# tjiangHIT/cuteSV

Measured on NVIDIA H100. Metric: sv_signatures_clustered_per_sec, higher is better.
Workload: dtype int32

## Files before the change

cutesv_b200/csrc/cutesv_b200.cu:

```cuda
#include <cuda_runtime.h>
#include <dlfcn.h>
#include <nccl.h>
#include <stdarg.h>
#include <stdio.h>
#include <stdlib.h>
#include <string.h>

#include <algorithm>
#include <atomic>
#include <string>
#include <vector>

#include "../../include/cutesv_b200.h"
#include "core.h"
#include "devprims.cuh"
#include "host_tables.h"
#include "kernels.cuh"
#include "radix.cuh"
#include "extract.cuh"
#include "scan_core.h"
#include "sa_core.h"

using namespace csv;

// ... 932 lines not shown
    return CSV_OK;
}
template <typename K>
static int lane_sort(csv_ctx* c, Lane& L, bool iota, int64_t n, int bits, K** keys_out, uint32_t** vals_out) {
    return radix_sort<K>(c, L.stream, L.hist, c->lb, L.lb_status, true, L.keys_a.as<K>(), L.vals_a.as<uint32_t>(), L.keys_b.as<K>(),
                         L.vals_b.as<uint32_t>(), iota, n, bits, keys_out, vals_out);
}

static ClusterParams cluster_params(const csv_params& P, int t) {
    ClusterParams C;
    C.min_support = P.min_support;
    C.min_support_allele = P.min_support_allele;
    C.min_size = P.min_size;
    C.max_size = P.max_size;
    C.bias = t == CSV_DEL ? P.bias_del : t == CSV_INS ? P.bias_ins : t == CSV_INV ? P.bias_inv : t == CSV_DUP ? P.bias_dup : P.bias_tra;
    C.ratio = t == CSV_DEL ? P.ratio_del : t == CSV_INS ? P.ratio_ins : P.ratio_tra;
    C.keep = P.remain_reads_ratio > 1 ? 1 : P.remain_reads_ratio;
    C.genotype = P.genotype;
    return C;
}

static Emit make_emit(csv_ctx* c) {
    Emit E;
    E.cand = c->cand_tmp.as<csv_cand>();
    E.names = c->names.as<int32_t>();
    E.cnt = c->cnt.as<uint32_t>();
    E.ctr = c->counters.as<Counters>();
    E.pow_half = c->pow_half.as<double>();
    E.lim.cap_cand = c->cap_cand;
    E.lim.cap_names = c->cap_names;
    E.lim.pow_n = c->pow_n;
    E.cursor = c->emit_cursor.as<unsigned long long>();
    return E;
}

static int run_segment_and_cluster(csv_ctx* c, Lane& L, TypeJob& J, int t, uint32_t kslot_base) {
    Counters* ctr = c->counters.as<Counters>();
    const cudaStream_t s = L.stream;
    stage_begin(c, s, CSV_ST_SEGMENT);
    J.kslot_base = kslot_base;
    J.kept_start = c->kept[t].as<uint32_t>();
    J.big_list = L.big_list.as<uint32_t>();
    J.giant_list = L.giant_list.as<uint32_t>();
    J.giant_arena = L.giant_arena.as<char>();
    J.big_cap = (uint32_t)(L.big_list.cap / 4);
    J.giant_cap = (uint32_t)(L.giant_list.cap / 4);
    TileSync ts;
    int rc = make_sync(c->lb, L.lb_status, s, (size_t)(J.n_host / SEL_TILE + 2), &ts);
    if (rc) return rc;
    if ((J.cp.min_support + 31) / 32 + 1 <= HEAD_MAX_NEED_WORDS) {
        MemberRec MR;
        memset(&MR, 0, sizeof(MR));
        J.small_list = nullptr; J.n_small = nullptr; J.rest_list = nullptr; J.n_rest = nullptr; J.n_rest_lo = nullptr;
        if ((t == CSV_DEL || t == CSV_INS) && J.iv.rec) {
            MR.rec = const_cast<IndelRec*>(J.iv.rec); MR.recc = const_cast<int32_t*>(J.iv.recc);
            MR.a = J.iv.a; MR.b = J.iv.b; MR.rid = J.iv.rid; MR.c = J.iv.recc ? J.iv.c : nullptr; MR.sidx = J.iv.sidx;
            if (t == CSV_DEL && J.keys32) { MR.del_off = c->d_off.as<uint64_t>(); MR.n_contigs = c->n_contigs; }
            if (J.cp.keep >= 1.0 && J.small_path) {
                CU(L.rest_list.ensure((size_t)c->kept_cap[t] * 12 + 64));
                MR.rest_list = L.rest_list.as<uint32_t>();
                MR.small_list = (uint2*)(L.rest_list.as<uint32_t>() + c->kept_cap[t] + (c->kept_cap[t] & 1u));
                if ((rc = take_ticket(c->lb, &MR.n_small)) || (rc = take_ticket(c->lb, &MR.n_rest)) || (rc = take_ticket(c->lb, &MR.n_rest_lo)))
                    return rc;
                MR.rest_cap = c->kept_cap[t];
                J.small_list = MR.small_list; J.n_small = MR.n_small; J.rest_list = MR.rest_list; J.n_rest = MR.n_rest;
                J.n_rest_lo = MR.n_rest_lo; J.rest_cap = MR.rest_cap;
            }
        }
        const int sel_grid = std::min(grid_for(c, J.n_host, SEL_TILE, 64), resident_grid(c, k_select_heads, SEL_THREADS, 0));
        if (L.prev_is_chain_kernel)
            LAUNCH_PDL(c, s, k_select_heads, sel_grid, SEL_THREADS, 0, J, c->kept[t].as<uint32_t>(), c->kept_cap[t],
                       &ctr->n_kept[t], ts, &ctr->status, (uint32_t)ST_LIST_OVERFLOW, MR);
        else
            LAUNCH(c, s, k_select_heads, sel_grid, SEL_THREADS, 0, J, c->kept[t].as<uint32_t>(), c->kept_cap[t],
                   &ctr->n_kept[t], ts, &ctr->status, (uint32_t)ST_LIST_OVERFLOW, MR);
    } else {
        J.iv.rec = nullptr; J.iv.recc = nullptr;
        HeadPred hp{J};
        LAUNCH(c, s, (k_select<HeadPred>), grid_for(c, J.n_host, SEL_TILE, 4), SEL_THREADS, 0, hp, J.n_host, J.n_dev,
               c->kept[t].as<uint32_t>(), c->kept_cap[t], &ctr->n_kept[t], ts, &ctr->status, (uint32_t)ST_LIST_OVERFLOW);
    }
    stage_end(c, s, CSV_ST_SEGMENT);
    stage_begin(c, s, CSV_ST_CLUSTER);
    Emit E = make_emit(c);
    const size_t smem_warp = (size_t)(CL_THREADS / 32) * WARP_M * ARENA_PER_MAX + (CL_THREADS / 32) * 40 * 8;
    uint32_t* work = nullptr;
    if ((rc = take_ticket(c->lb, &work))) return rc;
    const bool keep_all = J.cp.keep >= 1.0;
    const int side_k = t == CSV_INS ? 1 : 0;
    cudaStream_t gs = s;
    if (kind_of(t) == 0 && keep_all && J.small_path) {
        uint32_t* work_s = nullptr;
        if ((rc = take_ticket(c->lb, &work_s))) return rc;
        TypeJob JS = J;
        uint32_t* n_rest = nullptr;
        if (!J.small_list) {
            CU(L.rest_list.ensure((size_t)c->kept_cap[t] * 12 + 64));
            if ((rc = take_ticket(c->lb, &n_rest))) return rc;
            JS.rest_list = L.rest_list.as<uint32_t>();
            JS.n_rest = n_rest;
        } else if (!c->profiling) {
            gs = c->side_stream[side_k];
            CU(cudaEventRecord(c->ev_side_fork[side_k], s));
            CU(cudaStreamWaitEvent(gs, c->ev_side_fork[side_k], 0));
        }
        if (t == CSV_INS) LAUNCH_PDL_NAMED(c, s, "k_cluster_small<INS>", (k_cluster_small<true>), c->n_sm * 6, 256, 0, JS, E, ctr, work_s, n_rest);
        else LAUNCH_PDL_NAMED(c, s, "k_cluster_small<DEL>", (k_cluster_small<false>), c->n_sm * 6, 256, 0, JS, E, ctr, work_s, n_rest);
        if (!J.small_list) { J.rest_list = JS.rest_list; J.n_rest = n_rest; }
    } else { J.small_list = nullptr; J.n_small = nullptr; J.rest_list = nullptr; J.n_rest = nullptr; J.n_rest_lo = nullptr; }
    switch (kind_of(t)) {
        case 0:
            if (t == CSV_DEL) { if (keep_all) launch_cluster_kind<6, 0>(c, gs, J, E, ctr, work, smem_warp); else launch_cluster_kind<4, 0>(c, gs, J, E, ctr, work, smem_warp); }
            else { if (keep_all) launch_cluster_kind<7, 0>(c, gs, J, E, ctr, work, smem_warp); else launch_cluster_kind<5, 0>(c, gs, J, E, ctr, work, smem_warp); }
            break;
        case 1: launch_cluster_kind<1, 1>(c, gs, J, E, ctr, work, smem_warp); break;
        case 2: launch_cluster_kind<2, 2>(c, gs, J, E, ctr, work, smem_warp); break;
        default: launch_cluster_kind<3, 3>(c, gs, J, E, ctr, work, smem_warp); break;
    }
    if (gs != s) {
        CU(cudaEventRecord(c->ev_side_join[side_k], gs));
        CU(cudaStreamWaitEvent(s, c->ev_side_join[side_k], 0));
    }
    stage_end(c, s, CSV_ST_CLUSTER);
    if (L.mark >= 0) { CU(cudaEventRecord(c->kivs[L.mark].b, s)); L.mark = -1; }
    return CSV_OK;
}

static int run_indel(csv_ctx* c, Lane& L, int t, uint32_t kslot_base) {
    SigTable& s = c->sig[t];
    const cudaStream_t st = L.stream;
    const int64_t n = s.n;
    const uint64_t total = c->contig_off[c->n_contigs];
    const int bits = bits_for(total);
    const bool k64 = bits > 32;
    ContigTab ct{c->d_off.as<uint64_t>(), c->d_len_eff.as<int64_t>(), c->n_contigs};
    Counters* ctr = c->counters.as<Counters>();
    TypeJob J;
    memset(&J, 0, sizeof(J));
    J.svtype = t; J.n_host = n; J.n_dev = nullptr;
    J.cp = cluster_params(c->P, t);
    const uint32_t radius = (uint32_t)std::min<int64_t>((int64_t)(J.cp.min_support - 1) * J.cp.bias, 1 << 24);
    const double lambda = (double)n * (2.0 * radius + 2.0 * (1 << BKT_SHIFT)) / (double)std::max<uint64_t>(total, 1);
    const int rb = (int)((radius + (1u << BKT_SHIFT) - 1) >> BKT_SHIFT);
    const bool prefilter = !k64 && c->prefilter_enabled && J.cp.min_support >= 3 && lambda < 0.8 * J.cp.min_support &&
                           n >= (1 << 16) && rb <= BKT_PAD;
    J.iv.rec = nullptr; J.iv.recc = nullptr;
    uint32_t* sidx = nullptr;
    int rc;
    if (prefilter) {
        int W = PART_W_MAX;
        while (W > PART_W_MIN && (int64_t)(total >> W) + 1 < 2 * (int64_t)c->n_sm) W--;
        const int P = (int)(total >> W) + 1;
        const int n_chunks = (int)((n + PART_ROUND - 1) / PART_ROUND);
        const size_t run_words = (size_t)(P + 1) * n_chunks, edge_words = (size_t)P * 2 * BKT_PAD;
        stage_begin(c, st, CSV_ST_KEYS);
        CU(L.boff.ensure((run_words + edge_words) * 4));
        uint32_t* runs = L.boff.as<uint32_t>();
        uint32_t* edge = runs + run_words;
        CU(L.rec_a.ensure((size_t)n * sizeof(IndelRec)));
        CU(cudaMemsetAsync(edge, 0, edge_words * 4, st));
        const int is_ins = t == CSV_INS ? 1 : 0;
        if ((((uintptr_t)s.chrom.p) | ((uintptr_t)s.a.p)) & 15)
            return set_err(CSV_E_STATE, "signature columns are not 16 B aligned");
        uint2* pairs = (uint2*)L.keys_a.p;
        LAUNCH(c, st, k_part_scatter, n_chunks, PS_THREADS, ps_smem_bytes(), s.chrom.as<int32_t>(), s.a.as<int32_t>(), n, is_ins, ct, W, P,
               n_chunks, rb, pairs, runs, edge, &ctr->status);
        stage_end(c, st, CSV_ST_KEYS);
        stage_begin(c, st, CSV_ST_SORT);
        TileSync ts;
        rc = make_sync(c->lb, L.lb_status, st, (size_t)P, &ts);
        if (rc) return rc;
        uint32_t* n_pass = &ctr->n_dom[t];
        const size_t smem = pf_smem_bytes(W);
        const int g = std::min(P, resident_grid(c, k_part_filter, 256, smem));
        LAUNCH_PDL(c, st, k_part_filter, g, 256, smem, (const uint2*)pairs, (const uint32_t*)runs, n_chunks, P, W, rb, (uint32_t)J.cp.min_support,
                   (const uint32_t*)edge, L.keys_b.as<uint32_t>(), L.vals_b.as<uint32_t>(), (uint2*)L.rec_a.p, n_pass, ts);
        stage_end(c, st, CSV_ST_SORT);
        if (c->lane_marks) {
            kprof_begin(c, st, t == CSV_DEL ? "back end<DEL>" : "back end<INS>");
            L.mark = (int)c->kivs.size() - 1;
        }
        J.n_dev = n_pass;
        J.keys32 = L.keys_b.as<uint32_t>();
        sidx = L.vals_b.as<uint32_t>();
    } else {
        stage_begin(c, st, CSV_ST_KEYS);
        if (!k64)
            LAUNCH(c, st, (k_indel_keys<uint32_t>), grid_for(c, n, 256), 256, 0, s.chrom.as<int32_t>(), s.a.as<int32_t>(), s.b.as<int32_t>(),
                   s.rid.as<int32_t>(), n, t == CSV_INS ? 1 : 0, ct, L.keys_a.as<uint32_t>(), &ctr->status);
        else
            LAUNCH(c, st, (k_indel_keys<uint64_t>), grid_for(c, n, 256), 256, 0, s.chrom.as<int32_t>(), s.a.as<int32_t>(), s.b.as<int32_t>(),
                   s.rid.as<int32_t>(), n, t == CSV_INS ? 1 : 0, ct, L.keys_a.as<uint64_t>(), &ctr->status);
        stage_end(c, st, CSV_ST_KEYS);
        stage_begin(c, st, CSV_ST_SORT);
        if (!k64) {
            uint32_t* ko = nullptr;
            rc = lane_sort<uint32_t>(c, L, true, n, bits, &ko, &sidx);
            J.keys32 = ko;
        } else {
            uint64_t* ko = nullptr;
            rc = lane_sort<uint64_t>(c, L, true, n, bits, &ko, &sidx);
            J.keys64 = ko;
        }
        if (rc) return rc;
        stage_end(c, st, CSV_ST_SORT);
    }
    J.iv.chrom = s.chrom.as<int32_t>(); J.iv.a = s.a.as<int32_t>(); J.iv.b = s.b.as<int32_t>(); J.iv.rid = s.rid.as<int32_t>();
    J.iv.c = s.has_c ? s.c.as<int32_t>() : nullptr;
    J.iv.sidx = sidx;
    if (!k64 && c->records_enabled && (J.cp.min_support + 31) / 32 + 1 <= HEAD_MAX_NEED_WORDS) {
        const bool with_c = t == CSV_INS && s.has_c;
        CU(L.rec_a.ensure((size_t)n * sizeof(IndelRec)));
        if (with_c) CU(L.recc_a.ensure((size_t)n * 4));
        J.iv.rec = L.rec_a.as<IndelRec>();
        J.iv.recc = with_c ? L.recc_a.as<int32_t>() : nullptr;
    }
    J.iv.is_ins = t == CSV_INS ? 1 : 0;
    J.small_path = c->small_path_enabled ? 1 : 0;
    L.prev_is_chain_kernel = prefilter;
    rc = run_segment_and_cluster(c, L, J, t, kslot_base);
    L.prev_is_chain_kernel = false;
    return rc;
}

static int run_other(csv_ctx* c, Lane& L, int t, uint32_t kslot_base) {
    SigTable& s = c->sig[t];
    const cudaStream_t st = L.stream;
    const int64_t n = s.n;
    SmallWork& w = L.small;
    ContigTab ct{c->d_off.as<uint64_t>(), c->d_len_eff.as<int64_t>(), c->n_contigs};
    Counters* ctr = c->counters.as<Counters>();
    const uint64_t hi_max = t == CSV_DUP ? (uint64_t)c->n_contigs : t == CSV_INV ? 2ull * c->n_contigs : 4ull * c->n_contigs * c->n_contigs;
    const int clog = c->n_contigs > 1 ? bits_for((uint64_t)c->n_contigs - 1) : 0;
    const bool compact = t == CSV_TRA && 2 * clog + 33 > 64;
    const int prim_bits = 31 + bits_for(compact ? (uint64_t)n : hi_max);
    const int32_t* col_c = s.has_c ? s.c.as<int32_t>() : nullptr;
    const bool chain = c->small_chain[t];
    uint64_t* k_prim = chain ? w.k_prim.as<uint64_t>() : L.keys_a.as<uint64_t>();
    int rc;
    stage_begin(c, st, CSV_ST_KEYS);
    if (!compact) {
        LAUNCH(c, st, (k_other_keys<false>), grid_for(c, n, 256), 256, 0, s.chrom.as<int32_t>(), s.a.as<int32_t>(), s.b.as<int32_t>(),
               s.rid.as<int32_t>(), col_c, n, t, ct, chain ? w.k_rid.as<uint32_t>() : (uint32_t*)nullptr, w.k_b.as<uint32_t>(), k_prim,
               &ctr->status);
    } else {
        LAUNCH(c, st, (k_other_keys<true>), grid_for(c, n, 256), 256, 0, s.chrom.as<int32_t>(), s.a.as<int32_t>(), s.b.as<int32_t>(),
               s.rid.as<int32_t>(), col_c, n, t, ct, chain ? w.k_rid.as<uint32_t>() : (uint32_t*)nullptr, w.k_b.as<uint32_t>(),
               L.keys_a.as<uint64_t>(), &ctr->status);
        uint64_t* pair_sorted = nullptr;
        uint32_t* pair_perm = nullptr;
        rc = lane_sort<uint64_t>(c, L, true, n, bits_for(hi_max), &pair_sorted, &pair_perm);
        if (rc) return rc;
        uint32_t* rank = w.sel.as<uint32_t>();
        LAUNCH(c, st, k_tra_pair_flags, grid_for(c, n, 256), 256, 0, (const uint64_t*)pair_sorted, n, rank);
        TileSync ts;
        rc = make_sync(c->lb, L.lb_status, st, (size_t)(n / (SEL_THREADS * 4) + 2), &ts);
        if (rc) return rc;
        LAUNCH(c, st, (k_scan_excl<4>), grid_for(c, n, SEL_THREADS * 4, 4), SEL_THREADS, 0, rank, n, (const uint32_t*)nullptr,
               (const uint32_t*)nullptr, (uint32_t*)nullptr, ts);
        LAUNCH(c, st, k_tra_compact_key, grid_for(c, n, 256), 256, 0, (const uint32_t*)pair_perm, (const uint32_t*)rank, s.a.as<int32_t>(), n,
               k_prim);
    }
    stage_end(c, st, CSV_ST_KEYS);
    stage_begin(c, st, CSV_ST_SORT);
    if (!chain) {
        uint64_t* k64o = nullptr;
        uint32_t* perm = nullptr;
        rc = lane_sort<uint64_t>(c, L, true, n, prim_bits, &k64o, &perm);
        if (rc) return rc;
        LAUNCH(c, st, k_run_fixup, grid_for(c, n, 256), 256, 0, k64o, perm, n, s.b.as<int32_t>(), s.rid.as<int32_t>(), w.perm_b.as<uint32_t>(),
               &ctr->status);
    } else {
        uint32_t *k32o = nullptr, *perm = nullptr;
        LAUNCH(c, st, (k_gather_keys<uint32_t>), grid_for(c, n, 256), 256, 0, w.k_rid.as<uint32_t>(), (const uint32_t*)nullptr, n, L.keys_a.as<uint32_t>());
        rc = lane_sort<uint32_t>(c, L, true, n, 31, &k32o, &perm);
        if (rc) return rc;
        CU(cudaMemcpyAsync(w.perm_a.p, perm, (size_t)n * 4, cudaMemcpyDeviceToDevice, st));
        LAUNCH(c, st, (k_gather_keys<uint32_t>), grid_for(c, n, 256), 256, 0, w.k_b.as<uint32_t>(), w.perm_a.as<uint32_t>(), n, L.keys_a.as<uint32_t>());
        CU(cudaMemcpyAsync(L.vals_a.p, w.perm_a.p, (size_t)n * 4, cudaMemcpyDeviceToDevice, st));
        rc = lane_sort<uint32_t>(c, L, false, n, 31, &k32o, &perm);
        if (rc) return rc;
        CU(cudaMemcpyAsync(w.perm_a.p, perm, (size_t)n * 4, cudaMemcpyDeviceToDevice, st));
        LAUNCH(c, st, (k_gather_keys<uint64_t>), grid_for(c, n, 256), 256, 0, w.k_prim.as<uint64_t>(), w.perm_a.as<uint32_t>(), n, L.keys_a.as<uint64_t>());
        CU(cudaMemcpyAsync(L.vals_a.p, w.perm_a.p, (size_t)n * 4, cudaMemcpyDeviceToDevice, st));
        uint64_t* k64o = nullptr;
        rc = lane_sort<uint64_t>(c, L, false, n, prim_bits, &k64o, &perm);
        if (rc) return rc;
        CU(cudaMemcpyAsync(w.perm_b.p, perm, (size_t)n * 4, cudaMemcpyDeviceToDevice, st));
    }
    stage_end(c, st, CSV_ST_SORT);
    stage_begin(c, st, CSV_ST_SEGMENT);
    uint32_t* n_u = &ctr->n_dom[t];
    TileSync ts;
    rc = make_sync(c->lb, L.lb_status, st, (size_t)(n / SEL_TILE + 2), &ts);
    if (rc) return rc;
    DedupPred dp{s.chrom.as<int32_t>(), s.a.as<int32_t>(), s.b.as<int32_t>(), s.rid.as<int32_t>(), col_c, w.perm_b.as<uint32_t>()};
    LAUNCH(c, st, (k_select<DedupPred>), grid_for(c, n, SEL_TILE, 4), SEL_THREADS, 0, dp, n, (const uint32_t*)nullptr, w.sel.as<uint32_t>(),
           (uint32_t)n, n_u, ts, &ctr->status, (uint32_t)ST_INTERNAL);
    LAUNCH(c, st, k_other_gather, grid_for(c, n, 256), 256, 0, s.chrom.as<int32_t>(), s.a.as<int32_t>(), s.b.as<int32_t>(), s.rid.as<int32_t>(),
           col_c, w.perm_b.as<uint32_t>(), w.sel.as<uint32_t>(), n_u, w.u_chrom.as<int32_t>(), w.u_a.as<int32_t>(), w.u_b.as<int32_t>(),
           w.u_rid.as<int32_t>(), w.u_c.as<int32_t>());
    stage_end(c, st, CSV_ST_SEGMENT);
    TypeJob J;
    memset(&J, 0, sizeof(J));
    J.svtype = t; J.n_host = n; J.n_dev = n_u;
    J.cp = cluster_params(c->P, t);
    J.sv.chrom = w.u_chrom.as<int32_t>(); J.sv.a = w.u_a.as<int32_t>(); J.sv.b = w.u_b.as<int32_t>();
    J.sv.rid = w.u_rid.as<int32_t>(); J.sv.c = w.u_c.as<int32_t>();
    return run_segment_and_cluster(c, L, J, t, kslot_base);
}

static int ensure_small(Lane& L, size_t ns) {
    SmallWork& w = L.small;
    CU(w.k_rid.ensure(ns * 4)); CU(w.k_b.ensure(ns * 4)); CU(w.k_prim.ensure(ns * 8)); CU(w.perm_a.ensure(ns * 4)); CU(w.perm_b.ensure(ns * 4));
    CU(w.sel.ensure(ns * 4)); CU(w.u_chrom.ensure(ns * 4)); CU(w.u_a.ensure(ns * 4)); CU(w.u_b.ensure(ns * 4)); CU(w.u_rid.ensure(ns * 4));
    CU(w.u_c.ensure(ns * 4));
    return CSV_OK;
}
static int ensure_lane_scratch(Lane& L, size_t nm) {
    CU(L.keys_a.ensure(nm * 8)); CU(L.keys_b.ensure(nm * 8)); CU(L.vals_a.ensure(nm * 4)); CU(L.vals_b.ensure(nm * 4));
    CU(L.big_list.ensure((nm / WARP_M + 2) * 4));
    CU(L.giant_list.ensure((nm / BLOCK_M + 2) * 4));
    CU(L.giant_arena.ensure(nm * 2 * ARENA_PER_MAX + 256));
    return CSV_OK;
}

static int ensure_workspace(csv_ctx* c, uint32_t type_mask) {
    int64_t n_max = 0, n_total = 0, n_small_max = 0;
// ... 437 lines not shown
```

cutesv_b200/csrc/kernels.cuh:

```cuda
#pragma once
#include "core.h"
#include "devprims.cuh"
#include "radix.cuh"
#include <type_traits>

namespace csv {

static constexpr int WARP_M = 128;
static constexpr int BLOCK_M = 2048;
static constexpr int CL_THREADS = 256;

struct TypeJob {
    int svtype;
    int64_t n_host;
    const uint32_t* n_dev;
    const uint32_t* keys32;
    const uint64_t* keys64;
    IndelView iv;
    SortedView sv;
    ClusterParams cp;
    uint32_t kslot_base;
    const uint32_t* kept_start;
    uint32_t* big_list;
    uint32_t* giant_list;
// ... 141 lines not shown
#pragma unroll
                for (int u = 0; u < GATHER_GROUP; u++)
                    if (mem >> (j0 + u) & 1u) x[u] = sidx[base + threadIdx.x + (j0 + u) * SEL_THREADS];
#pragma unroll
                for (int u = 0; u < GATHER_GROUP; u++) {
                    if (mem >> (j0 + u) & 1u) {
                        const int64_t i = base + threadIdx.x + (j0 + u) * SEL_THREADS;
                        IndelRec r;
                        r.a = aoff != ~0u ? (int32_t)(J.keys32[i] - aoff) : ca[x[u]];
                        r.b = cb[x[u]]; r.rid = cr[x[u]]; r.idx = x[u];
                        const int32_t c5 = cc ? cc[x[u]] : 0;
                        if (r.rid < 0 || r.b < 0 || c5 < 0) bad |= ST_NEG_FIELD;
                        *reinterpret_cast<int4*>(&rec[i]) = *reinterpret_cast<const int4*>(&r);
                        if (recc) recc[i] = c5;
                    }
                }
            }
            if (bad) atomicOr(status_word, bad);
        }
        __syncthreads();
        uint32_t o = s_excl + local;
#pragma unroll
        for (int j = 0; j < SEL_ITEMS; j++) {
            if (flags >> j & 1u) {
                if (o < out_cap) out[o] = (uint32_t)(base + p0 + j);
                else atomicOr(status_word, overflow_bit);
                o++;
            }
        }
        if (MR.small_list) {
            const uint32_t ex = s_excl;
            for (uint32_t h0 = warp * 32; h0 < total; h0 += SEL_THREADS) {
                const uint32_t h = h0 + lane;
                const uint32_t sz = h < total ? s_msize[h] : 255u;
                const uint32_t lt = (1u << lane) - 1u;
                const uint32_t m_small = __ballot_sync(0xffffffffu, sz <= 32u);
                const uint32_t m_lo = __ballot_sync(0xffffffffu, sz == 33u), m_hi = __ballot_sync(0xffffffffu, sz == 34u);
                uint32_t b_small = 0, b_lo = 0, b_hi = 0;
                if (lane == 0) {
                    if (m_small) b_small = atomicAdd(MR.n_small, (uint32_t)__popc(m_small));
                    if (m_lo) b_lo = atomicAdd(MR.n_rest_lo, (uint32_t)__popc(m_lo));
                    if (m_hi) b_hi = atomicAdd(MR.n_rest, (uint32_t)__popc(m_hi));
                }
                b_small = __shfl_sync(0xffffffffu, b_small, 0);
                b_lo = __shfl_sync(0xffffffffu, b_lo, 0);
                b_hi = __shfl_sync(0xffffffffu, b_hi, 0);
                if (sz <= 32u) MR.small_list[b_small + __popc(m_small & lt)] = make_uint2(ex + h, sz);
                else if (sz == 33u) MR.rest_list[MR.rest_cap - 1u - (b_lo + __popc(m_lo & lt))] = ex + h;
                else if (sz == 34u) MR.rest_list[b_hi + __popc(m_hi & lt)] = ex + h;
            }
        }
        __syncthreads();
    }
}

struct ContigTab {
    const uint64_t* off;
    const int64_t* len;
    int32_t n;
};

static constexpr int BKT_SHIFT = 8;
static constexpr int BKT_PAD = 64;

__global__ void __launch_bounds__(256) k_check_contig_off(const int64_t* __restrict__ off, int n_contigs, int64_t n, uint32_t* bad) {
    bool ok = true;
    for (int64_t k = (int64_t)blockIdx.x * blockDim.x + threadIdx.x; k <= n_contigs; k += (int64_t)gridDim.x * blockDim.x) {
        const int64_t o = off[k];
        if (k == 0 && o != 0) ok = false;
        if (k == n_contigs && o != n) ok = false;
        if (k < n_contigs && off[k + 1] < o) ok = false;
    }
    if (!ok) atomicOr(bad, ST_BAD_GROUPS);
}
__global__ void k_fold_status(const uint32_t* __restrict__ src, uint32_t* dst) {
    if (threadIdx.x == 0 && *src) atomicOr(dst, *src);
}

__global__ void __launch_bounds__(256) k_expand_contigs(const int64_t* __restrict__ off, int n_contigs, int64_t n, int32_t* __restrict__ chrom,
                                                        const uint32_t* __restrict__ bad) {
    if (bad && *bad) {
        for (int64_t i = (int64_t)blockIdx.x * blockDim.x + threadIdx.x; i < n; i += (int64_t)gridDim.x * blockDim.x) chrom[i] = 0;
        return;
    }
    for (int64_t v = (int64_t)blockIdx.x * blockDim.x + threadIdx.x; v * 4 < n; v += (int64_t)gridDim.x * blockDim.x) {
        const int64_t i0 = v * 4;
        int lo = 0, hi = n_contigs;
        while (hi - lo > 1) { const int mid = (lo + hi) >> 1; if (__ldg(&off[mid]) <= i0) lo = mid; else hi = mid; }
        int k = lo;
#pragma unroll
        for (int j = 0; j < 4; j++) {
            const int64_t i = i0 + j;
            if (i >= n) break;
            while (__ldg(&off[k + 1]) <= i) k++;
            chrom[i] = k;
        }
    }
}

template <typename K>
__global__ void __launch_bounds__(256) k_indel_keys(const int32_t* __restrict__ chrom, const int32_t* __restrict__ a, const int32_t* __restrict__ b,
                             const int32_t* __restrict__ rid, int64_t n, int is_ins, ContigTab ct, K* __restrict__ keys,
                             uint32_t* status) {
    auto one = [&](int32_t c, int32_t raw, int32_t bb, int32_t rr, uint32_t& bad) -> K {
        K key = 0;
        if (c < 0 || c >= ct.n) bad |= ST_BAD_CHROM;
        else {
            const int64_t pos = is_ins ? (raw >> 1) : raw;
            if (raw < 0 || pos > ct.len[c]) bad |= ST_BAD_POS;
            else key = (K)(ct.off[c] + (uint64_t)pos);
        }
        if (rr < 0 || bb < 0) bad |= ST_NEG_FIELD;
        return key;
    };
    const int64_t tid = (int64_t)blockIdx.x * blockDim.x + threadIdx.x, stride = (int64_t)gridDim.x * blockDim.x;
    const bool aligned = ((((uintptr_t)chrom) | ((uintptr_t)a) | ((uintptr_t)b) | ((uintptr_t)rid) | ((uintptr_t)keys)) & 15) == 0;
    const int64_t nv = aligned ? (n >> 2) : 0;
    uint32_t bad = 0;
    for (int64_t v = tid; v < nv; v += stride) {
        const int4 c4 = reinterpret_cast<const int4*>(chrom)[v], a4 = reinterpret_cast<const int4*>(a)[v];
        const int4 b4 = reinterpret_cast<const int4*>(b)[v], r4 = reinterpret_cast<const int4*>(rid)[v];
        const K k0 = one(c4.x, a4.x, b4.x, r4.x, bad), k1 = one(c4.y, a4.y, b4.y, r4.y, bad);
        const K k2 = one(c4.z, a4.z, b4.z, r4.z, bad), k3 = one(c4.w, a4.w, b4.w, r4.w, bad);
        if (sizeof(K) == 4) reinterpret_cast<uint4*>(keys)[v] = make_uint4((uint32_t)k0, (uint32_t)k1, (uint32_t)k2, (uint32_t)k3);
        else {
            reinterpret_cast<ulonglong2*>(keys)[2 * v] = make_ulonglong2((uint64_t)k0, (uint64_t)k1);
            reinterpret_cast<ulonglong2*>(keys)[2 * v + 1] = make_ulonglong2((uint64_t)k2, (uint64_t)k3);
        }
    }
    for (int64_t i = nv * 4 + tid; i < n; i += stride) {
        const K key = one(chrom[i], a[i], b[i], rid[i], bad);
        keys[i] = key;
    }
    if (bad) atomicOr(status, bad);
}

__device__ __forceinline__ uint32_t indel_key32(int32_t c, int32_t raw, int is_ins, const ContigTab& ct, uint32_t& bad) {
    if (c < 0 || c >= ct.n) { bad |= ST_BAD_CHROM; return 0u; }
    const int64_t pos = is_ins ? (raw >> 1) : raw;
    if (raw < 0 || pos > ct.len[c]) { bad |= ST_BAD_POS; return 0u; }
    return (uint32_t)(ct.off[c] + (uint64_t)pos);
}

static constexpr int PART_MAX = 1024;
static constexpr int PART_W_MAX = 22;
static constexpr int PART_W_MIN = 16;
static constexpr int PF_STAGE = 5632;
static constexpr int FIX_SMALL = 64;
static constexpr int PF_BIG_CAP = 256;
__host__ __device__ constexpr size_t pf_smem_bytes(int w) {
    return (size_t)(1u << (w - BKT_SHIFT)) * 4 + (size_t)(1u << (w - BKT_SHIFT)) / 32 * 4 + (size_t)PF_STAGE * 8;
}

static constexpr int PS_THREADS = 1024;
static constexpr int PART_ROUND = 16384, PART_ROUND_V = PART_ROUND / 4 / PS_THREADS;
__host__ __device__ constexpr size_t ps_smem_bytes() { return (size_t)PART_ROUND * 8 + (size_t)PART_MAX * 4; }
static_assert(PART_MAX == PS_THREADS && PART_ROUND % (4 * PS_THREADS) == 0, "k_part_scatter tiling: one partition per thread");
static_assert(ps_smem_bytes() + 256 <= 227 * 1024, "k_part_scatter: one round per SM");
__global__ void __launch_bounds__(PS_THREADS, 1) k_part_scatter(const int32_t* __restrict__ chrom, const int32_t* __restrict__ a, int64_t n,
                                                                int is_ins, ContigTab ct, int W, int P, int n_chunks, int rb,
                                                                uint2* __restrict__ pairs, uint32_t* __restrict__ runs,
                                                                uint32_t* __restrict__ edge, uint32_t* status) {
    pdl_launch_dependents();
    extern __shared__ __align__(16) uint32_t s_dyn[];
    uint2* s_st = reinterpret_cast<uint2*>(s_dyn);
    int32_t* s_c = reinterpret_cast<int32_t*>(s_dyn);
    int32_t* s_a = reinterpret_cast<int32_t*>(s_dyn) + PART_ROUND;
    uint32_t* s_fill = s_dyn + 2 * PART_ROUND;
    __shared__ uint32_t s_warp[32];
    __shared__ __align__(8) uint64_t s_bar;
    const int t = (int)threadIdx.x, lane = t & 31, warp = t >> 5;
    const int64_t s0 = (int64_t)blockIdx.x * PART_ROUND;
    const int m = (int)min((int64_t)PART_ROUND, n - s0);
    const int m4 = m & ~3;
    if (t == 0) {
        mbar_init(&s_bar, 1);
        asm volatile("fence.proxy.async.shared::cta;" ::: "memory");
        if (m4) {
            mbar_expect_tx(&s_bar, (uint32_t)m4 * 8);
            bulk_copy(s_c, chrom + s0, (uint32_t)m4 * 4, &s_bar);
            bulk_copy(s_a, a + s0, (uint32_t)m4 * 4, &s_bar);
        } else {
            mbar_arrive(&s_bar);
        }
    }
    if (m4 + t < m) { s_c[m4 + t] = chrom[s0 + m4 + t]; s_a[m4 + t] = a[s0 + m4 + t]; }
    s_fill[t] = 0;
    __syncthreads();
    mbar_wait(&s_bar, 0);
    uint32_t key[4 * PART_ROUND_V], bad = 0;
#pragma unroll
    for (int j = 0; j < PART_ROUND_V; j++) {
        const int r = 4 * (j * PS_THREADS + t);
        const int4 cv = reinterpret_cast<const int4*>(s_c)[j * PS_THREADS + t];
        const int4 av = reinterpret_cast<const int4*>(s_a)[j * PS_THREADS + t];
        uint32_t b0 = 0, b1 = 0, b2 = 0, b3 = 0;
        key[4 * j] = indel_key32(cv.x, av.x, is_ins, ct, b0);
        key[4 * j + 1] = indel_key32(cv.y, av.y, is_ins, ct, b1);
        key[4 * j + 2] = indel_key32(cv.z, av.z, is_ins, ct, b2);
        key[4 * j + 3] = indel_key32(cv.w, av.w, is_ins, ct, b3);
        bad |= (r < m ? b0 : 0u) | (r + 1 < m ? b1 : 0u) | (r + 2 < m ? b2 : 0u) | (r + 3 < m ? b3 : 0u);
    }
    if (bad) atomicOr(status, bad);
    const uint32_t bmask = (1u << (W - BKT_SHIFT)) - 1;
#pragma unroll
    for (int k = 0; k < 4 * PART_ROUND_V; k++) {
        if (4 * ((k >> 2) * PS_THREADS + t) + (k & 3) >= m) continue;
        const uint32_t p = key[k] >> W, bl = (key[k] >> BKT_SHIFT) & bmask;
        if (bl < (uint32_t)rb) atomicAdd(&edge[p * 2 * BKT_PAD + bl], 1u);
        if (bmask - bl < (uint32_t)rb) atomicAdd(&edge[p * 2 * BKT_PAD + BKT_PAD + (bmask - bl)], 1u);
        atomicAdd(&s_fill[p], 1u);
    }
    __syncthreads();
    {
        const uint32_t v = s_fill[t];
        uint32_t incl = v;
#pragma unroll
        for (int d = 1; d < 32; d <<= 1) {
            const uint32_t y = __shfl_up_sync(0xffffffffu, incl, d);
            if (lane >= d) incl += y;
        }
        if (lane == 31) s_warp[warp] = incl;
        __syncthreads();
        if (warp == 0) {
            const uint32_t w = s_warp[lane];
            uint32_t wi = w;
#pragma unroll
            for (int d = 1; d < 32; d <<= 1) {
                const uint32_t y = __shfl_up_sync(0xffffffffu, wi, d);
                if (lane >= d) wi += y;
            }
            s_warp[lane] = wi - w;
        }
        __syncthreads();
        const uint32_t o = s_warp[warp] + incl - v;
        s_fill[t] = o;
        if (t < P) runs[(int64_t)t * n_chunks + blockIdx.x] = o;
        if (t == 0) runs[(int64_t)P * n_chunks + blockIdx.x] = (uint32_t)m;
    }
    __syncthreads();
#pragma unroll
    for (int k = 0; k < 4 * PART_ROUND_V; k++) {
        const int q = 4 * ((k >> 2) * PS_THREADS + t) + (k & 3);
        if (q < m) s_st[atomicAdd(&s_fill[key[k] >> W], 1u)] = make_uint2(key[k], (uint32_t)(s0 + q));
    }
    __syncthreads();
    uint2* dst = pairs + s0;
    for (int q = t; q < (m >> 1); q += PS_THREADS) reinterpret_cast<uint4*>(dst)[q] = reinterpret_cast<const uint4*>(s_st)[q];
    if ((m & 1) && t == 0) dst[m - 1] = s_st[m - 1];
}

template <int U, class F>
__device__ __forceinline__ void part_walk_runs(const uint2* __restrict__ pairs, const uint32_t* __restrict__ runs, int p, int n_chunks,
                                               F f) {
    const int lane = threadIdx.x & 31;
    const uint32_t* r0 = runs + (int64_t)p * n_chunks;
    const uint32_t* r1 = r0 + n_chunks;
    const int TR = n_chunks >= 2 * 8 * 32 ? 32 : 16;
    const bool mine = lane < TR;
    int c = (int)(threadIdx.x >> 5) * TR + lane;
    uint32_t nb = 0, ne = 0;
    if (mine && c < n_chunks) { nb = __ldcg(r0 + c); ne = __ldcg(r1 + c); }
    for (; c - lane < n_chunks; c += 8 * TR) {
        const uint32_t len = ne - nb;
        uint32_t end = len;
#pragma unroll
        for (int d = 1; d < 32; d <<= 1) {
            const uint32_t v = __shfl_up_sync(0xffffffffu, end, d);
            if (lane >= d) end += v;
        }
        const uint32_t tot = __shfl_sync(0xffffffffu, end, 31);
        const uint32_t src = (uint32_t)c * PART_ROUND + nb - (end - len);
        nb = ne = 0;
        if (mine && c + 8 * TR < n_chunks) { nb = __ldcg(r0 + c + 8 * TR); ne = __ldcg(r1 + c + 8 * TR); }
        const uint32_t end15 = __shfl_sync(0xffffffffu, end, 15);
        for (uint32_t e0 = 0; e0 < tot; e0 += 32 * U) {
            uint32_t at[U];
#pragma unroll
            for (int u = 0; u < U; u++) {
                const uint32_t e = e0 + 32 * u + lane;
                int r = end15 <= e ? 16 : 0;
#pragma unroll
                for (int s = 8; s; s >>= 1) r += __shfl_sync(0xffffffffu, end, r + s - 1) <= e ? s : 0;
                at[u] = __shfl_sync(0xffffffffu, src, r) + e;
            }
            uint2 pr[U];
#pragma unroll
            for (int u = 0; u < U; u++) pr[u] = e0 + 32 * u + lane < tot ? pairs[at[u]] : make_uint2(0u, 0u);
#pragma unroll
            for (int u = 0; u < U; u++) f(pr[u], e0 + 32 * u + lane < tot);
        }
    }
}

__global__ void __launch_bounds__(256) k_part_filter(const uint2* __restrict__ pairs, const uint32_t* __restrict__ runs, int n_chunks, int P, int W, int rb,
                                                     uint32_t need, const uint32_t* __restrict__ edge, uint32_t* __restrict__ keys_out,
                                                     uint32_t* __restrict__ idx_out, uint2* __restrict__ spill, uint32_t* n_out, TileSync ts) {
    pdl_launch_dependents(); pdl_wait();
    extern __shared__ __align__(16) uint32_t s_dyn[];
    const int BP = 1 << (W - BKT_SHIFT), LPER = W - BKT_SHIFT - 8, PER = 1 << LPER;
    uint32_t* s_h = s_dyn;
    uint32_t* s_f = s_dyn + BP;
    uint2* s_st = reinterpret_cast<uint2*>(s_dyn + BP + BP / 32);
    __shared__ uint32_t s_warp[9];
    __shared__ uint32_t s_hl[BKT_PAD], s_hr[BKT_PAD];
    __shared__ uint32_t s_big[PF_BIG_CAP], s_cnt[256];
    __shared__ uint32_t s_tile, s_excl, s_nbig;
    const int lane = threadIdx.x & 31, warp = threadIdx.x >> 5;
    const uint32_t gen = ts_gen(ts);
    const uint32_t bmask = BP - 1;
    static_assert(PART_W_MIN - BKT_SHIFT >= 8 && PART_W_MAX - BKT_SHIFT <= 14, "one strip of 1..64 buckets per thread");
    auto phys = [&](uint32_t b) -> uint32_t { return ((b & (PER - 1)) << 8) | (b >> LPER); };
    auto count = [&](int b) -> uint32_t { return s_h[phys(b)]; };
    const int b0 = (int)threadIdx.x * PER;
    while (true) {
        if (threadIdx.x == 0) { s_tile = atomicAdd(ts.ticket, 1u); s_nbig = 0; }
        for (int i = threadIdx.x; i < BP; i += 256) s_h[i] = 0;
        __syncthreads();
        const int p = (int)s_tile;
        if (p >= P) break;
        if (threadIdx.x < 2 * BKT_PAD) {
            const int j = threadIdx.x % BKT_PAD, right = threadIdx.x / BKT_PAD;
            const int q = right ? p + 1 : p - 1;
            const bool ok = q >= 0 && q < P && j < rb;
            (right ? s_hr : s_hl)[j] = ok ? edge[(int64_t)q * 2 * BKT_PAD + (right ? 0 : BKT_PAD) + j] : 0u;
        }
        constexpr int U = 16;
        part_walk_runs<U>(pairs, runs, p, n_chunks, [&](uint2 pr, bool v) {
            if (v) atomicAdd(&s_h[phys((pr.x >> BKT_SHIFT) & bmask)], 1u);
        });
        __syncthreads();
        uint32_t kept, S;
        const uint64_t flags = pf_strip_flags(count, [&](int s, int j) -> uint32_t { return s_h[(j << 8) + (int)threadIdx.x + s]; },
                                              b0, PER, BP, rb, need, s_hl, s_hr, &kept);
        const uint32_t first = block_excl_scan_256(kept, s_warp, &S);
        if (threadIdx.x == 0) {
            lookback_publish(ts.status, gen, p, S);
            if (S) atomicAdd(n_out, S);
        }
        const bool spilled = S > (uint32_t)PF_STAGE;
        if (spilled && warp == 0) {
            const uint32_t ex = lookback_wait_warp(ts.status, gen, p, S);
            if (lane == 0) s_excl = ex;
        }
        pf_strip_offsets([&](int b) -> uint32_t { return s_h[((b - b0) << 8) | threadIdx.x]; }, b0, PER, flags, first,
                         [&](int j, uint32_t off, bool f, uint32_t c) {
            s_h[(j << 8) | threadIdx.x] = off;
            const uint32_t bits = __ballot_sync(0xffffffffu, f);
            if (lane == 0) s_f[(j << 3) | warp] = bits;
            if (c > FIX_SMALL) {
                const uint32_t q = atomicAdd(&s_nbig, 1u);
                if (q < PF_BIG_CAP) s_big[q] = (uint32_t)(b0 + j);
            }
        });
        __syncthreads();
        if (!spilled && warp == 0) {
            const uint32_t ex = lookback_wait_warp(ts.status, gen, p, S);
            if (lane == 0) s_excl = ex;
        }
        uint2* st = spilled ? spill + s_excl : s_st;
        part_walk_runs<U>(pairs, runs, p, n_chunks, [&](uint2 pr, bool v) {
            const uint32_t ph = phys((pr.x >> BKT_SHIFT) & bmask);
            if (v && ((s_f[ph >> 5] >> (ph & 31)) & 1u)) st[atomicAdd(&s_h[ph], 1u)] = pr;
        });
        __syncthreads();
        const uint32_t obase = s_excl;
        for (uint32_t q = threadIdx.x; q < S; q += 256) {
            const uint2 pr = st[q];
            const uint32_t b = (pr.x >> BKT_SHIFT) & bmask;
            const uint32_t beg = b ? s_h[phys(b - 1)] : 0u, end = s_h[phys(b)];
            if (end - beg > FIX_SMALL) continue;
            uint32_t rank = 0;
            for (uint32_t j = beg; j < end; j++) {
                const uint32_t k = st[j].x;
                rank += (k < pr.x || (k == pr.x && j < q)) ? 1u : 0u;
            }
            keys_out[obase + beg + rank] = pr.x;
            idx_out[obase + beg + rank] = pr.y;
        }
        static_assert((1 << BKT_SHIFT) == 256, "one counting-sort bin per thread");
        const uint32_t nbig = s_nbig;
        const uint32_t nb = nbig <= (uint32_t)PF_BIG_CAP ? nbig : (uint32_t)BP;
        for (uint32_t k = 0; k < nb; k++) {
            const uint32_t b = nbig <= (uint32_t)PF_BIG_CAP ? s_big[k] : k;
            const uint32_t beg = b ? s_h[phys(b - 1)] : 0u, end = s_h[phys(b)];
            if (end - beg <= FIX_SMALL) continue;
            __syncthreads();
            s_cnt[threadIdx.x] = 0;
            __syncthreads();
            for (uint32_t j = beg + threadIdx.x; j < end; j += 256) atomicAdd(&s_cnt[st[j].x & 255u], 1u);
            __syncthreads();
            uint32_t total;
            const uint32_t ex = block_excl_scan_256(s_cnt[threadIdx.x], s_warp, &total);
            s_cnt[threadIdx.x] = ex;
            __syncthreads();
            for (uint32_t j = beg + threadIdx.x; j < end; j += 256) {
                const uint2 pr = st[j];
                const uint32_t d = obase + beg + atomicAdd(&s_cnt[pr.x & 255u], 1u);
                keys_out[d] = pr.x;
                idx_out[d] = pr.y;
            }
        }
        __syncthreads();
    }
}

template <bool TRA_PAIR>
__global__ void k_other_keys(const int32_t* __restrict__ chrom, const int32_t* __restrict__ a, const int32_t* __restrict__ b,
                             const int32_t* __restrict__ rid, const int32_t* __restrict__ c, int64_t n, int svtype, ContigTab ct,
                             uint32_t* __restrict__ k_rid, uint32_t* __restrict__ k_b, uint64_t* __restrict__ k_prim,
                             uint32_t* status) {
    for (int64_t i = (int64_t)blockIdx.x * blockDim.x + threadIdx.x; i < n; i += (int64_t)gridDim.x * blockDim.x) {
        uint32_t bad = 0;
        const int32_t ch = chrom[i], ai = a[i], bi = b[i], ri = rid[i], ci = c ? c[i] : 0;
        if (ch < 0 || ch >= ct.n) bad |= ST_BAD_CHROM;
        else if (ct.len[ch] < 0) bad |= ST_BAD_POS;
        if (ai < 0 || bi < 0 || ri < 0 || ci < 0) bad |= ST_NEG_FIELD;
        if (svtype == CSV_TRA && (ci >> 2) >= ct.n) bad |= ST_BAD_CHROM;
        if (svtype == CSV_INV && ci > 1) bad |= ST_NEG_FIELD;
        if (bad) atomicOr(status, bad);
        if (k_rid) { k_rid[i] = (uint32_t)ri; k_b[i] = (uint32_t)bi; }
        uint64_t hi = (uint64_t)(uint32_t)ch;
        if (svtype == CSV_INV) hi = hi * 2 + (uint32_t)ci;
        if (svtype == CSV_TRA) hi = hi * (uint64_t)(4 * ct.n) + (uint32_t)ci;
        k_prim[i] = TRA_PAIR ? hi : (hi << 31) | (uint32_t)ai;
    }
}

__global__ void k_tra_pair_flags(const uint64_t* __restrict__ pair_sorted, int64_t n, uint32_t* __restrict__ flag) {
    for (int64_t i = (int64_t)blockIdx.x * blockDim.x + threadIdx.x; i < n; i += (int64_t)gridDim.x * blockDim.x)
        flag[i] = (i + 1 < n && pair_sorted[i + 1] != pair_sorted[i]) ? 1u : 0u;
}
__global__ void k_tra_compact_key(const uint32_t* __restrict__ perm, const uint32_t* __restrict__ rank, const int32_t* __restrict__ a,
                                  int64_t n, uint64_t* __restrict__ k_prim) {
    for (int64_t i = (int64_t)blockIdx.x * blockDim.x + threadIdx.x; i < n; i += (int64_t)gridDim.x * blockDim.x) {
        const uint32_t x = perm[i];
        k_prim[x] = ((uint64_t)rank[i] << 31) | (uint32_t)a[x];
    }
}

static constexpr int RUN_MAX = 2048;
__global__ void __launch_bounds__(256) k_run_fixup(const uint64_t* __restrict__ kprim_sorted, const uint32_t* __restrict__ perm, int64_t n,
                                                   const int32_t* __restrict__ b, const int32_t* __restrict__ rid,
                                                   uint32_t* __restrict__ perm_out, uint32_t* status) {
    for (int64_t i = (int64_t)blockIdx.x * blockDim.x + threadIdx.x; i < n; i += (int64_t)gridDim.x * blockDim.x) {
        const uint64_t k = kprim_sorted[i];
        const uint32_t x = perm[i];
        const bool alone = (i == 0 || kprim_sorted[i - 1] != k) && (i + 1 >= n || kprim_sorted[i + 1] != k);
        if (alone) { perm_out[i] = x; continue; }
        const int32_t bx = b[x], rx = rid[x];
        int64_t lo = i, hi = i + 1;
        uint32_t rank = 0;
        int seen = 1;
        auto less = [&](uint32_t y) { const int32_t by = b[y], ry = rid[y]; return by < bx || (by == bx && (ry < rx || (ry == rx && y < x))); };
        while (lo > 0 && kprim_sorted[lo - 1] == k && seen <= RUN_MAX) { rank += less(perm[lo - 1]) ? 1u : 0u; lo--; seen++; }
        while (hi < n && kprim_sorted[hi] == k && seen <= RUN_MAX) { rank += less(perm[hi]) ? 1u : 0u; hi++; seen++; }
        if (seen > RUN_MAX) { atomicOr(status, ST_BIG_RUN); perm_out[i] = x; continue; }
        perm_out[lo + rank] = x;
    }
}

template <typename K>
__global__ void k_gather_keys(const K* __restrict__ src, const uint32_t* __restrict__ perm, int64_t n, K* __restrict__ out) {
    for (int64_t i = (int64_t)blockIdx.x * blockDim.x + threadIdx.x; i < n; i += (int64_t)gridDim.x * blockDim.x)
        out[i] = src[perm ? perm[i] : (uint32_t)i];
}

struct DedupPred {
    const int32_t *chrom, *a, *b, *rid, *c;
    const uint32_t* perm;
    __device__ __forceinline__ bool operator()(int64_t i) const {
        if (i == 0) return true;
        const uint32_t x = perm[i], y = perm[i - 1];
        return !(chrom[x] == chrom[y] && a[x] == a[y] && b[x] == b[y] && rid[x] == rid[y] && (c ? c[x] == c[y] : true));
    }
};
__global__ void k_other_gather(const int32_t* __restrict__ chrom, const int32_t* __restrict__ a, const int32_t* __restrict__ b,
                               const int32_t* __restrict__ rid, const int32_t* __restrict__ c, const uint32_t* __restrict__ perm,
                               const uint32_t* __restrict__ sel, const uint32_t* n_sel, int32_t* u_chrom, int32_t* u_a, int32_t* u_b,
                               int32_t* u_rid, int32_t* u_c) {
    const int64_t n = *n_sel;
    for (int64_t k = (int64_t)blockIdx.x * blockDim.x + threadIdx.x; k < n; k += (int64_t)gridDim.x * blockDim.x) {
        const uint32_t x = perm[sel[k]];
        u_chrom[k] = chrom[x]; u_a[k] = a[x]; u_b[k] = b[x]; u_rid[k] = rid[x]; u_c[k] = c ? c[x] : 0;
    }
}

__host__ __device__ constexpr int kind_of(int svtype) { return (svtype == CSV_DEL || svtype == CSV_INS) ? 0 : svtype == CSV_DUP ? 1 : svtype == CSV_INV ? 2 : 3; }
template <int KIND, class Team>
__device__ __forceinline__ void run_cluster(Team tm, const TypeJob& J, int64_t s, int m, int M, char* arena, int64_t* red,
                                            uint32_t kslot, const Emit& E) {
    if (KIND == 4) indel_cluster<Team, CSV_DEL, 0>(tm, J.iv, s, m, M, arena, red, J.cp, J.svtype, kslot, E);
    else if (KIND == 5) indel_cluster<Team, CSV_INS, 0>(tm, J.iv, s, m, M, arena, red, J.cp, J.svtype, kslot, E);
    else if (KIND == 6) indel_cluster<Team, CSV_DEL, 1>(tm, J.iv, s, m, M, arena, red, J.cp, J.svtype, kslot, E);
    else if (KIND == 7) indel_cluster<Team, CSV_INS, 1>(tm, J.iv, s, m, M, arena, red, J.cp, J.svtype, kslot, E);
    else if (KIND == 0) indel_cluster(tm, J.iv, s, m, M, arena, red, J.cp, J.svtype, kslot, E);
    else if (KIND == 1) dup_cluster(tm, J.sv, s, m, M, arena, red, J.cp, kslot, E);
    else if (KIND == 2) inv_cluster(tm, J.sv, s, m, M, arena, red, J.cp, kslot, E);
    else tra_cluster(tm, J.sv, s, m, M, arena, red, J.cp, kslot, E);
}
__device__ __forceinline__ int arena_per(const TypeJob& J) {
    return (J.svtype == CSV_DEL || J.svtype == CSV_INS) ? INDEL_ARENA_PER : OTHER_ARENA_PER;
}
static constexpr int ARENA_PER_MAX = INDEL_ARENA_PER > OTHER_ARENA_PER ? INDEL_ARENA_PER : OTHER_ARENA_PER;

__device__ __forceinline__ int cluster_size_warp(const TypeJob& J, int64_t s, int64_t n, int limit) {
    const int lane = threadIdx.x & 31;
    int m = 1;
    while (m <= limit) {
        const int64_t i = s + m + lane;
        const bool brk = (i >= n) || !job_linked(J, i);
        const uint32_t mask = __ballot_sync(0xffffffffu, brk);
        if (mask) { m += __ffs(mask) - 1; return m; }
        m += 32;
    }
    return m;
}

// ... 797 lines not shown
```

Before: 18.94 billion.

## Scatter partition pairs into paged per-partition pools instead of per-chunk runs

Replaces the per-chunk sorted runs plus run-offset table with a paged pool. Each partition gets a page table filled by atomically allocated 2048-pair pages, so k_part_scatter writes pairs straight into contiguous per-partition pages. k_part_filter can then stream each partition with coalesced 16-byte loads instead of walking many small runs with shuffle-based searches. The cost is global atomics, a cross-block spin-wait on shared lead pages, and page tables that must be reset after use.

Result: faster. 19.94 billion (median of 6 runs) (+5.3%).

```diff
diff --git a/cutesv_b200/csrc/cutesv_b200.cu b/cutesv_b200/csrc/cutesv_b200.cu
--- a/cutesv_b200/csrc/cutesv_b200.cu
+++ b/cutesv_b200/csrc/cutesv_b200.cu
@@ -1108,28 +1108,31 @@
         while (W > PART_W_MIN && (int64_t)(total >> W) + 1 < 2 * (int64_t)c->n_sm) W--;
         const int P = (int)(total >> W) + 1;
         const int n_chunks = (int)((n + PART_ROUND - 1) / PART_ROUND);
-        const size_t run_words = (size_t)(P + 1) * n_chunks, edge_words = (size_t)P * 2 * BKT_PAD;
+        const uint32_t ptw = (uint32_t)((n + PART_PAGE - 1) / PART_PAGE) + 1;
+        const size_t edge_words = (size_t)PART_MAX * 2 * BKT_PAD, tab_words = PART_MAX + (size_t)P * ptw;
         stage_begin(c, st, CSV_ST_KEYS);
-        CU(L.boff.ensure((run_words + edge_words) * 4));
-        uint32_t* runs = L.boff.as<uint32_t>();
-        uint32_t* edge = runs + run_words;
+        CU(L.boff.ensure((edge_words + tab_words) * 4, true));
+        uint32_t* edge = L.boff.as<uint32_t>();
+        uint32_t* fill = edge + edge_words;
+        uint32_t* pt = fill + PART_MAX;
+        CU(L.keys_a.ensure(((size_t)ptw - 1 + P) * PART_PAGE * 8));
+        uint2* pool = (uint2*)L.keys_a.p;
         CU(L.rec_a.ensure((size_t)n * sizeof(IndelRec)));
-        CU(cudaMemsetAsync(edge, 0, edge_words * 4, st));
+        CU(cudaMemsetAsync(edge, 0, (size_t)P * 2 * BKT_PAD * 4, st));
         const int is_ins = t == CSV_INS ? 1 : 0;
         if ((((uintptr_t)s.chrom.p) | ((uintptr_t)s.a.p)) & 15)
             return set_err(CSV_E_STATE, "signature columns are not 16 B aligned");
-        uint2* pairs = (uint2*)L.keys_a.p;
+        uint32_t* pool_next = nullptr;
+        TileSync ts;
+        if ((rc = take_ticket(c->lb, &pool_next)) || (rc = make_sync(c->lb, L.lb_status, st, (size_t)P, &ts))) return rc;
+        const size_t smem = pf_smem_bytes(W);
+        const int g = std::min(P, resident_grid(c, k_part_filter, 256, smem));
         LAUNCH(c, st, k_part_scatter, n_chunks, PS_THREADS, ps_smem_bytes(), s.chrom.as<int32_t>(), s.a.as<int32_t>(), n, is_ins, ct, W, P,
-               n_chunks, rb, pairs, runs, edge, &ctr->status);
+               rb, pool, fill, pt, ptw, pool_next, edge, &ctr->status);
         stage_end(c, st, CSV_ST_KEYS);
         stage_begin(c, st, CSV_ST_SORT);
-        TileSync ts;
-        rc = make_sync(c->lb, L.lb_status, st, (size_t)P, &ts);
-        if (rc) return rc;
         uint32_t* n_pass = &ctr->n_dom[t];
-        const size_t smem = pf_smem_bytes(W);
-        const int g = std::min(P, resident_grid(c, k_part_filter, 256, smem));
-        LAUNCH_PDL(c, st, k_part_filter, g, 256, smem, (const uint2*)pairs, (const uint32_t*)runs, n_chunks, P, W, rb, (uint32_t)J.cp.min_support,
+        LAUNCH_PDL(c, st, k_part_filter, g, 256, smem, (const uint2*)pool, fill, pt, ptw, P, W, rb, (uint32_t)J.cp.min_support,
                    (const uint32_t*)edge, L.keys_b.as<uint32_t>(), L.vals_b.as<uint32_t>(), (uint2*)L.rec_a.p, n_pass, ts);
         stage_end(c, st, CSV_ST_SORT);
         if (c->lane_marks) {
diff --git a/cutesv_b200/csrc/kernels.cuh b/cutesv_b200/csrc/kernels.cuh
--- a/cutesv_b200/csrc/kernels.cuh
+++ b/cutesv_b200/csrc/kernels.cuh
@@ -317,22 +317,30 @@
     return (size_t)(1u << (w - BKT_SHIFT)) * 4 + (size_t)(1u << (w - BKT_SHIFT)) / 32 * 4 + (size_t)PF_STAGE * 8;
 }
 
+static constexpr int PART_PAGE = 2048;
+static_assert(PART_PAGE % 2 == 0, "k_part_filter reads pairs two at a time, 16 B aligned");
+
 static constexpr int PS_THREADS = 1024;
 static constexpr int PART_ROUND = 16384, PART_ROUND_V = PART_ROUND / 4 / PS_THREADS;
-__host__ __device__ constexpr size_t ps_smem_bytes() { return (size_t)PART_ROUND * 8 + (size_t)PART_MAX * 4; }
+static constexpr int PS_PAGES = PART_ROUND / PART_PAGE + 2 * PART_MAX;
+__host__ __device__ constexpr size_t ps_smem_bytes() { return (size_t)PART_ROUND * 8 + (size_t)PART_MAX * 4 * 3 + (size_t)PS_PAGES * 4; }
 static_assert(PART_MAX == PS_THREADS && PART_ROUND % (4 * PS_THREADS) == 0, "k_part_scatter tiling: one partition per thread");
 static_assert(ps_smem_bytes() + 256 <= 227 * 1024, "k_part_scatter: one round per SM");
 __global__ void __launch_bounds__(PS_THREADS, 1) k_part_scatter(const int32_t* __restrict__ chrom, const int32_t* __restrict__ a, int64_t n,
-                                                                int is_ins, ContigTab ct, int W, int P, int n_chunks, int rb,
-                                                                uint2* __restrict__ pairs, uint32_t* __restrict__ runs,
-                                                                uint32_t* __restrict__ edge, uint32_t* status) {
+                                                                int is_ins, ContigTab ct, int W, int P, int rb, uint2* __restrict__ pool,
+                                                                uint32_t* __restrict__ fill, uint32_t* pt, uint32_t ptw,
+                                                                uint32_t* __restrict__ pool_next, uint32_t* __restrict__ edge,
+                                                                uint32_t* status) {
     pdl_launch_dependents();
     extern __shared__ __align__(16) uint32_t s_dyn[];
     uint2* s_st = reinterpret_cast<uint2*>(s_dyn);
     int32_t* s_c = reinterpret_cast<int32_t*>(s_dyn);
     int32_t* s_a = reinterpret_cast<int32_t*>(s_dyn) + PART_ROUND;
     uint32_t* s_fill = s_dyn + 2 * PART_ROUND;
-    __shared__ uint32_t s_warp[32];
+    uint32_t* s_d = s_fill + PART_MAX;
+    uint32_t* s_pb = s_d + PART_MAX;
+    uint32_t* s_pg = s_pb + PART_MAX;
+    __shared__ uint32_t s_warp[32], s_npg;
     __shared__ __align__(8) uint64_t s_bar;
     const int t = (int)threadIdx.x, lane = t & 31, warp = t >> 5;
     const int64_t s0 = (int64_t)blockIdx.x * PART_ROUND;
@@ -348,6 +356,7 @@
         } else {
             mbar_arrive(&s_bar);
         }
+        s_npg = 0;
     }
     if (m4 + t < m) { s_c[m4 + t] = chrom[s0 + m4 + t]; s_a[m4 + t] = a[s0 + m4 + t]; }
     s_fill[t] = 0;
@@ -377,8 +386,9 @@
         atomicAdd(&s_fill[p], 1u);
     }
     __syncthreads();
+    const uint32_t v = s_fill[t];
+    const uint32_t r = v ? atomicAdd(&fill[t], v) : 0u;
     {
-        const uint32_t v = s_fill[t];
         uint32_t incl = v;
 #pragma unroll
         for (int d = 1; d < 32; d <<= 1) {
@@ -400,66 +410,56 @@
         __syncthreads();
         const uint32_t o = s_warp[warp] + incl - v;
         s_fill[t] = o;
-        if (t < P) runs[(int64_t)t * n_chunks + blockIdx.x] = o;
-        if (t == 0) runs[(int64_t)P * n_chunks + blockIdx.x] = (uint32_t)m;
-    }
+        s_d[t] = r - o;
+    }
+    const uint32_t k0 = r / PART_PAGE, k1 = v ? (r + v - 1) / PART_PAGE : k0;
+    const bool lead = v && r % PART_PAGE != 0;
+    const uint32_t np = v ? k1 - k0 + 1 : 0u, own = np - (lead ? 1u : 0u);
+    uint32_t* row = pt + (size_t)t * ptw;
+    const uint32_t id = own ? atomicAdd(pool_next, own) : 0u;
+    uint32_t g = 1;
+    if (lead) asm volatile("ld.relaxed.gpu.global.u32 %0, [%1];" : "=r"(g) : "l"(row + k0) : "memory");
+    uint32_t base = np;
+#pragma unroll
+    for (int d = 1; d < 32; d <<= 1) {
+        const uint32_t y = __shfl_up_sync(0xffffffffu, base, d);
+        if (lane >= d) base += y;
+    }
+    uint32_t wbase = 0;
+    if (lane == 31) wbase = atomicAdd(&s_npg, base);
+    base = __shfl_sync(0xffffffffu, wbase, 31) + base - np;
+    s_pb[t] = base - k0;
     __syncthreads();
 #pragma unroll
     for (int k = 0; k < 4 * PART_ROUND_V; k++) {
         const int q = 4 * ((k >> 2) * PS_THREADS + t) + (k & 3);
         if (q < m) s_st[atomicAdd(&s_fill[key[k] >> W], 1u)] = make_uint2(key[k], (uint32_t)(s0 + q));
     }
+    for (uint32_t i = 0; i < own; i++) {
+        const uint32_t k = k1 + 1 - own + i;
+        asm volatile("st.relaxed.gpu.global.u32 [%0], %1;" ::"l"(row + k), "r"(id + i + 1u) : "memory");
+        s_pg[base + k - k0] = id + i;
+    }
+    if (lead) {
+        while (g == 0) {
+            __nanosleep(64);
+            asm volatile("ld.relaxed.gpu.global.u32 %0, [%1];" : "=r"(g) : "l"(row + k0) : "memory");
+        }
+        s_pg[base] = g - 1u;
+    }
     __syncthreads();
-    uint2* dst = pairs + s0;
-    for (int q = t; q < (m >> 1); q += PS_THREADS) reinterpret_cast<uint4*>(dst)[q] = reinterpret_cast<const uint4*>(s_st)[q];
-    if ((m & 1) && t == 0) dst[m - 1] = s_st[m - 1];
-}
-
-template <int U, class F>
-__device__ __forceinline__ void part_walk_runs(const uint2* __restrict__ pairs, const uint32_t* __restrict__ runs, int p, int n_chunks,
-                                               F f) {
-    const int lane = threadIdx.x & 31;
-    const uint32_t* r0 = runs + (int64_t)p * n_chunks;
-    const uint32_t* r1 = r0 + n_chunks;
-    const int TR = n_chunks >= 2 * 8 * 32 ? 32 : 16;
-    const bool mine = lane < TR;
-    int c = (int)(threadIdx.x >> 5) * TR + lane;
-    uint32_t nb = 0, ne = 0;
-    if (mine && c < n_chunks) { nb = __ldcg(r0 + c); ne = __ldcg(r1 + c); }
-    for (; c - lane < n_chunks; c += 8 * TR) {
-        const uint32_t len = ne - nb;
-        uint32_t end = len;
-#pragma unroll
-        for (int d = 1; d < 32; d <<= 1) {
-            const uint32_t v = __shfl_up_sync(0xffffffffu, end, d);
-            if (lane >= d) end += v;
-        }
-        const uint32_t tot = __shfl_sync(0xffffffffu, end, 31);
-        const uint32_t src = (uint32_t)c * PART_ROUND + nb - (end - len);
-        nb = ne = 0;
-        if (mine && c + 8 * TR < n_chunks) { nb = __ldcg(r0 + c + 8 * TR); ne = __ldcg(r1 + c + 8 * TR); }
-        const uint32_t end15 = __shfl_sync(0xffffffffu, end, 15);
-        for (uint32_t e0 = 0; e0 < tot; e0 += 32 * U) {
-            uint32_t at[U];
-#pragma unroll
-            for (int u = 0; u < U; u++) {
-                const uint32_t e = e0 + 32 * u + lane;
-                int r = end15 <= e ? 16 : 0;
-#pragma unroll
-                for (int s = 8; s; s >>= 1) r += __shfl_sync(0xffffffffu, end, r + s - 1) <= e ? s : 0;
-                at[u] = __shfl_sync(0xffffffffu, src, r) + e;
-            }
-            uint2 pr[U];
-#pragma unroll
-            for (int u = 0; u < U; u++) pr[u] = e0 + 32 * u + lane < tot ? pairs[at[u]] : make_uint2(0u, 0u);
-#pragma unroll
-            for (int u = 0; u < U; u++) f(pr[u], e0 + 32 * u + lane < tot);
-        }
-    }
-}
-
-__global__ void __launch_bounds__(256) k_part_filter(const uint2* __restrict__ pairs, const uint32_t* __restrict__ runs, int n_chunks, int P, int W, int rb,
-                                                     uint32_t need, const uint32_t* __restrict__ edge, uint32_t* __restrict__ keys_out,
+#pragma unroll
+    for (int j = 0; j < PART_ROUND / PS_THREADS; j++) {
+        const int q = j * PS_THREADS + t;
+        if (q >= m) break;
+        const uint2 pr = s_st[q];
+        const uint32_t p = pr.x >> W, e = (uint32_t)q + s_d[p];
+        pool[(size_t)s_pg[s_pb[p] + e / PART_PAGE] * PART_PAGE + e % PART_PAGE] = pr;
+    }
+}
+
+__global__ void __launch_bounds__(256) k_part_filter(const uint2* __restrict__ pool, uint32_t* __restrict__ fill, uint32_t* __restrict__ pt,
+                                                     uint32_t ptw, int P, int W, int rb, uint32_t need, const uint32_t* __restrict__ edge, uint32_t* __restrict__ keys_out,
                                                      uint32_t* __restrict__ idx_out, uint2* __restrict__ spill, uint32_t* n_out, TileSync ts) {
     pdl_launch_dependents(); pdl_wait();
     extern __shared__ __align__(16) uint32_t s_dyn[];
@@ -490,10 +490,31 @@
             const bool ok = q >= 0 && q < P && j < rb;
             (right ? s_hr : s_hl)[j] = ok ? edge[(int64_t)q * 2 * BKT_PAD + (right ? 0 : BKT_PAD) + j] : 0u;
         }
-        constexpr int U = 16;
-        part_walk_runs<U>(pairs, runs, p, n_chunks, [&](uint2 pr, bool v) {
-            if (v) atomicAdd(&s_h[phys((pr.x >> BKT_SHIFT) & bmask)], 1u);
-        });
+        const uint32_t np = __ldcg(fill + p);
+        uint32_t* row = pt + (size_t)p * ptw;
+        auto walk = [&](auto f) {
+            constexpr int U = 8;
+            static_assert(2 * 256 * U == 2 * PART_PAGE, "k_part_filter: two pages per step");
+            for (uint32_t k = 0; 2 * PART_PAGE * k < np; k++) {
+                const uint32_t e0 = 2 * PART_PAGE * k + 2 * threadIdx.x;
+                const uint2* pg0 = pool + (size_t)(__ldg(row + 2 * k) - 1u) * PART_PAGE;
+                const uint2* pg1 = PART_PAGE * (2 * k + 1) < np ? pool + (size_t)(__ldg(row + 2 * k + 1) - 1u) * PART_PAGE : pg0;
+                uint4 v[U];
+#pragma unroll
+                for (int u = 0; u < U; u++) {
+                    const uint32_t e = e0 + 2 * 256 * u;
+                    v[u] = e < np ? __ldg(reinterpret_cast<const uint4*>((2 * 256 * u + 2 * threadIdx.x < PART_PAGE ? pg0 : pg1) + e % PART_PAGE))
+                                  : make_uint4(0u, 0u, 0u, 0u);
+                }
+#pragma unroll
+                for (int u = 0; u < U; u++) {
+                    const uint32_t e = e0 + 2 * 256 * u;
+                    if (e < np) f(make_uint2(v[u].x, v[u].y));
+                    if (e + 1 < np) f(make_uint2(v[u].z, v[u].w));
+                }
+            }
+        };
+        walk([&](uint2 pr) { atomicAdd(&s_h[phys((pr.x >> BKT_SHIFT) & bmask)], 1u); });
         __syncthreads();
         uint32_t kept, S;
         const uint64_t flags = pf_strip_flags(count, [&](int s, int j) -> uint32_t { return s_h[(j << 8) + (int)threadIdx.x + s]; },
@@ -524,11 +545,13 @@
             if (lane == 0) s_excl = ex;
         }
         uint2* st = spilled ? spill + s_excl : s_st;
-        part_walk_runs<U>(pairs, runs, p, n_chunks, [&](uint2 pr, bool v) {
+        walk([&](uint2 pr) {
             const uint32_t ph = phys((pr.x >> BKT_SHIFT) & bmask);
-            if (v && ((s_f[ph >> 5] >> (ph & 31)) & 1u)) st[atomicAdd(&s_h[ph], 1u)] = pr;
+            if ((s_f[ph >> 5] >> (ph & 31)) & 1u) st[atomicAdd(&s_h[ph], 1u)] = pr;
         });
         __syncthreads();
+        for (uint32_t k = threadIdx.x; k < (np + PART_PAGE - 1) / PART_PAGE; k += 256) row[k] = 0u;
+        if (threadIdx.x == 0) fill[p] = 0u;
         const uint32_t obase = s_excl;
         for (uint32_t q = threadIdx.x; q < S; q += 256) {
             const uint2 pr = st[q];
```
